# Bissmella/Small-object-detection-transformers

Hardware: AMD Instinct MI355X
Metric: images/sec (1024x1024 RGB+IR) train fwd+bwd (higher is better)
Workload: dtype bf16; 1 GPU; SRyolo_MF.yaml (model.yaml graph), batch 8/GPU @ 1024x1024 RGB+IR, fwd + hand-written bwd + fused SGD-nesterov/weight-decay + EMA step, loss = YOLOv5 ComputeLoss (CIoU + BCE, device kernels), 32 synthetic boxes/image, random-init weights; global_batch=8, parallelism=dp1

## Files before the change

include/sodt_hip.h:

```cpp
#ifndef SODT_HIP_H
#define SODT_HIP_H
#include <stddef.h>
#include <stdint.h>

#ifdef __cplusplus
extern "C" {
#endif

typedef struct ihipStream_t* sodt_stream_t;

#define SODT_OK 0
#define SODT_EINVAL 1
#define SODT_ELAUNCH 2

#define SODT_F32 0
#define SODT_BF16 1
#define SODT_MAX_SEG 9

typedef struct {
  const void* p;
  int ld;
  int klen;
  int dy, dx;
  int mul, shr;
  int Hi, Wi;
} sodt_seg;

typedef struct {
  sodt_seg s[SODT_MAX_SEG];
  int nseg;
  int spatial;
  int Ho, Wo;
} sodt_aspec;

#define SODT_EPI_BIAS 1
#define SODT_EPI_RESID 2
#define SODT_EPI_GELU_DUAL 4
#define SODT_EPI_DGELU 8
#define SODT_EPI_STATS 16
#define SODT_STATS_REPL 16
#define SODT_EPI_AFFINE_SILU 32
#define SODT_EPI_DETECT 64
#define SODT_EPI_OUT_F32 128
#define SODT_EPI_GELU 256
#define SODT_EPI_DGELU_RC 512
#define SODT_EPI_RELU 2048
#define SODT_EPI_DRELU 4096

typedef struct {
  sodt_aspec a;
  const void* W; int ldw;
  void* C; int ldc;
  void* C2; int ldc2;
  const float* bias;
  const void* R; int ldr; int rmod;
  const void* aux; int ldaux;
  double* stats;
  const float* scale; const float* shift;
  int M, N, K, flags;
  int oscatter, omul, ody, odx, OH, OW;
  int det_na, det_no, det_hw;
} sodt_gemm_args;

int sodt_gemm_nt(const sodt_gemm_args* g, int dtype, sodt_stream_t st);
#define SODT_VARIANT_AUTO 0
#define SODT_VARIANT_TILED 1
#define SODT_VARIANT_ASTAT 2
#define SODT_VARIANT_NO_TN3 3
int sodt_gemm_set_variant(int variant);

typedef struct {
  const void* dY; int ldy;
  sodt_aspec x;
  float* dW; int lddw;
  float* dbias;
  int M, N, K;
  int kperm_c, kperm_t;
  int splits;
  float* partial;
  long partial_floats;
} sodt_gemm_tn_args;

int sodt_gemm_tn(const sodt_gemm_tn_args* g, int dtype, sodt_stream_t st);

typedef struct {
  const void* dY; int ldy;
  const void* X; int ldx;
  const void* wT; int ldw;
  const void* aux; int ldaux;
  void* dX; int lddx;
  float* dW; int lddw;
  float* dbias;
  int M, N, K, flags;
  int splits;
  float* partial;
  long partial_floats;
} sodt_linbwd_args;

int sodt_linear_bwd_sq(const sodt_linbwd_args* g, int dtype, sodt_stream_t st);

int sodt_layernorm_fwd(const void* x, const float* gamma, const float* beta, void* y, float* stats,
                       int M, int C, int dtype, sodt_stream_t st);
int sodt_layernorm_bwd(const void* dy, const void* x, const float* stats, const float* gamma,
                       const void* dres, void* dx, float* dgamma, float* dbeta,
                       int M, int C, int dtype, sodt_stream_t st);

int sodt_window_attn_fwd(const void* qkv, const float* bias_t, void* out, float* lse,
                         int B, int H, int W, int C, int heads, int ws, int shift,
                         int dtype, sodt_stream_t st);
int sodt_window_attn_bwd(const void* qkv, const float* bias_t, const void* out, const void* dout,
                         const float* lse, void* dqkv, float* dbias_t, float* dq_acc,
                         int B, int H, int W, int C, int heads, int ws, int shift,
                         int dtype, sodt_stream_t st);

int sodt_window_attn_sp_fwd(const void* qkv, const float* qkv_bias, const float* bias_t, void* out, float* lse,
                            int B, int H, int W, int C, int heads, int ws, int shift, int dtype, sodt_stream_t st);
int sodt_window_attn_sp_bwd(const void* qkv, const float* qkv_bias, const float* bias_t, const void* out, const void* dout,
                            const float* lse, void* dqkv, float* dqkv_bias, float* dbias_t,
                            int B, int H, int W, int C, int heads, int ws, int shift, int dtype, sodt_stream_t st);

int sodt_bilinear_up2_fwd(const void* x, void* y, int ldy, int B, int H, int W, int C, int dtype, sodt_stream_t st);
int sodt_bilinear_up2_bwd(const void* dy, int lddy, void* dx, const void* relu_out, int B, int H, int W, int C, int dtype,
                          sodt_stream_t st);
int sodt_pixel_shuffle2(const void* in, void* out, int B, int H, int W, int C, int inverse, int dtype, sodt_stream_t st);
int sodt_add_rows(void* dst, int ldd, int dcol, const void* src, int lds, int scol, long M, int C, int dtype, sodt_stream_t st);
int sodt_nchw_f32_from_rows(const void* rows, int ld, float* y, int B, int C, int H, int W, int dtype, sodt_stream_t st);
int sodt_rows_from_nchw_f32(const float* y, void* rows, int ld, int B, int C, int H, int W, int dtype, sodt_stream_t st);

int sodt_conv3x3_c64n8_fwd(const void* x, const void* w, const float* bias, void* y, float* y_nchw, int B, int H, int W, int cout, int dtype,
                           sodt_stream_t st);
int sodt_conv3x3_c64n8_dgrad(const void* dy, const float* dy_nchw, const void* wT, void* dx, int B, int H, int W, int cout, int dtype,
                             sodt_stream_t st);
int sodt_conv3x3_c64n8_wgrad(const void* dy, const float* dy_nchw, const void* x, float* dw, float* db, float* scratch, int B, int H, int W,
                             int cout, int dtype, sodt_stream_t st);
long sodt_conv3x3_c64n8_wgrad_scratch_bytes(void);

typedef struct {
  int w_row_stride, w_row_off;
  int in_mul, in_i, in_j;
  int out_mul, out_i, out_j;
} sodt_conv3_geo;
int sodt_conv3x3_c64_fwd(const void* x, const void* w, const float* bias, const void* resid, const void* aux, void* y, int B, int H, int W,
                         int flags, int flip, const sodt_conv3_geo* geo, int dtype, sodt_stream_t st);
int sodt_conv3x3_c64_wgrad(const void* dy, const void* x, float* dw, float* db, float* scratch, int B, int H, int W, const sodt_conv3_geo* geo,
                           int dtype, sodt_stream_t st);
long sodt_conv3x3_c64_wgrad_scratch_bytes(void);

long sodt_wmsa_pack_bytes(int C, int heads, int ws, int dtype);
int sodt_wmsa_pack(const float* qkv_w, const float* qkv_b, const float* proj_w, const float* proj_b,
                   const float* rpb_table, const float* n1_w, const float* n1_b, const float* n2_w,
                   const float* n2_b, void* wpk, int C, int heads, int ws, int dtype, sodt_stream_t st);
// ... 227 lines not shown
```

small-object-detection-transformers_amd/csrc/gemm.hip:

```cpp
#include "gemm_epi.h"
#include "launch.h"
#include "routes.h"

int sodt_nt3_launch(const sodt_gemm_args* g, const NtRoute& r, hipStream_t st);
int sodt_tn3_launch(const sodt_gemm_tn_args* g, const TnRoute& r, hipStream_t st);

namespace {

int g_variant = SODT_VARIANT_AUTO;

constexpr int BM = 128, BN = 128, ROWB = 128;
constexpr int STAGE_BYTES = BM * ROWB;
constexpr int EPI_LD = 132;
constexpr int NT_LDS = BM * EPI_LD * 4;


__device__ __forceinline__ sodt_seg pick_seg(const sodt_aspec& a, int i) {
  sodt_seg s = a.s[0];
#pragma unroll
  for (int j = 1; j < SODT_MAX_SEG; ++j)
    if (i == j) s = a.s[j];
  return s;
}


template <typename T, int CF>
__global__ __launch_bounds__(256, 2) void gemm_nt_kernel(const sodt_gemm_args g) {
  constexpr int KPL = TT<T>::KPL;
  constexpr int BK = 8 * KPL;
  constexpr int SZ = TT<T>::SZ;
  __shared__ __attribute__((aligned(16))) unsigned char smem[NT_LDS];
  unsigned char* sA = smem;
  unsigned char* sB = smem + 2 * STAGE_BYTES;
  __shared__ sodt_seg sSeg[SODT_MAX_SEG];

  const int tid = threadIdx.x, lane = tid & 63, wid = tid >> 6;
  if (tid == 0) {
#pragma unroll
    for (int j = 0; j < SODT_MAX_SEG; ++j) sSeg[j] = g.a.s[j];
  }
  __syncthreads();
  const int wr = wid >> 1, wc = wid & 1;
  const int ntn = (g.N + BN - 1) / BN;
  const int tile = xcd_remap(blockIdx.x, gridDim.x);
  const int tn = tile % ntn, tm = tile / ntn;
  const long m0 = (long)tm * BM;
  const int n0 = tn * BN;

  const int lrow = tid >> 3, lch = tid & 7;
  RowGeo geo[4];
  const int hw = g.a.Ho * g.a.Wo;
#pragma unroll
  for (int i = 0; i < 4; ++i) {
    const long m = m0 + lrow + 32 * i;
    geo[i].ok = m < g.M;
    geo[i].b = 0; geo[i].y = 0; geo[i].x = 0;
    if (g.a.spatial && geo[i].ok) {
      const int b = (int)(m / hw), rem = (int)(m - (long)b * hw);
      geo[i].b = b; geo[i].y = rem / g.a.Wo; geo[i].x = rem - geo[i].y * g.a.Wo;
    }
  }
  int a_seg = 0, a_off = lch * KPL;
  sodt_seg seg = g.a.s[0];
  long srow[4];
#pragma unroll
  for (int i = 0; i < 4; ++i) srow[i] = seg_src_row(seg, geo[i], g.a.spatial, m0 + lrow + 32 * i);

  uint4 ra[4], rb[4];
  const int nk = (g.K + BK - 1) / BK;

  auto load_regs = [&](int kt) {
    while (a_seg < g.a.nseg && a_off >= seg.klen) {
      a_off -= seg.klen;
      ++a_seg;
      if (a_seg < g.a.nseg) {
        seg = sSeg[a_seg];
#pragma unroll
        for (int i = 0; i < 4; ++i) srow[i] = seg_src_row(seg, geo[i], g.a.spatial, m0 + lrow + 32 * i);
      }
    }
    const bool kin = a_seg < g.a.nseg;
    const T* ap = (const T*)seg.p;
#pragma unroll
    for (int i = 0; i < 4; ++i) {
      ra[i] = make_uint4(0, 0, 0, 0);
      if (kin && srow[i] >= 0) ra[i] = *(const uint4*)(ap + srow[i] * seg.ld + a_off);
    }
    a_off += BK;
    const int k = kt * BK + lch * KPL;
    const T* wp = (const T*)g.W;
#pragma unroll
    for (int i = 0; i < 4; ++i) {
      const int n = n0 + lrow + 32 * i;
// ... 800 lines not shown
      }
    }
}

template <typename T>
int launch_tn2(const sodt_gemm_tn_args* g, hipStream_t st) {
  constexpr int lds = 2 * TN2Geo<T>::BMS * (TN2Geo<T>::YROW + TN2Geo<T>::XROW);
  const int tiles = ((g->N + 255) / 256) * ((g->K + 191) / 192);
  return sodt_launch<gemm_tn2_kernel<T>>(dim3(tiles * g->splits), dim3(512), lds, st, *g);
}

bool aspec_ok(const sodt_aspec& a, int K, int kpl) {
  if (a.nseg < 1 || a.nseg > SODT_MAX_SEG) return false;
  long tot = 0;
  for (int i = 0; i < a.nseg; ++i) {
    const sodt_seg& s = a.s[i];
    if (s.klen <= 0 || (s.klen % kpl) || (s.ld % kpl) || (((uintptr_t)s.p) & 15)) return false;
    if (a.spatial && (s.Hi <= 0 || s.Wi <= 0 || s.mul < 1 || s.shr < 0)) return false;
    tot += s.klen;
  }
  if (a.spatial && (a.Ho <= 0 || a.Wo <= 0)) return false;
  return tot == K;
}

#define NT_STATIC_CF(X) \
  X(0) X(SODT_EPI_BIAS) X(SODT_EPI_RESID) X(SODT_EPI_BIAS | SODT_EPI_RESID) X(SODT_EPI_BIAS | SODT_EPI_GELU_DUAL) X(SODT_EPI_DGELU)

template <typename T>
int launch_nt(const sodt_gemm_args* g, const NtRoute& r, hipStream_t st) {
  switch (r.kind) {
    case NT_REFUSED: return SODT_EINVAL;
    case NT_PIPE: return sodt_nt3_launch(g, r, st);
    case NT_BS_STATS: return launch_bs<T, 128, true, -1, false>(g, st);
    case NT_BS_SIMPLE:
      switch (r.cf) {
#define X(F) case F: return launch_bs<T, 128, false, F, true>(g, st);
        NT_STATIC_CF(X)
#undef X
      }
      return SODT_EINVAL;
    case NT_BS_GENERIC: return launch_bs<T, 128, false, -1, false>(g, st);
    case NT_AS128: return launch_as<T, 128>(g, st);
    case NT_AS64: return launch_as<T, 64>(g, st);
    case NT_TILED: {
      const long tiles = ((long)(g->M + BM - 1) / BM) * ((g->N + BN - 1) / BN);
      if (tiles > 0x7fffffffL) return SODT_EINVAL;
      const dim3 grid((unsigned)tiles), block(256);
      switch (r.cf) {
#define X(F) case F: return sodt_launch<gemm_nt_kernel<T, F>>(grid, block, 0, st, *g);
        NT_STATIC_CF(X)
#undef X
      }
      return sodt_launch<gemm_nt_kernel<T, -1>>(grid, block, 0, st, *g);
    }
  }
  return SODT_EINVAL;
}
#undef NT_STATIC_CF

}

extern "C" int sodt_gemm_nt(const sodt_gemm_args* g, int dtype, sodt_stream_t st) {
  if (!g || g->M <= 0 || g->N <= 0 || g->K <= 0 || (dtype != SODT_BF16 && dtype != SODT_F32)) return SODT_EINVAL;
  const int kpl = dtype == SODT_BF16 ? 8 : 4;
  if (!aspec_ok(g->a, g->K, kpl)) return SODT_EINVAL;
  if ((g->ldw % kpl) || (((uintptr_t)g->W) & 15) || !g->C) return SODT_EINVAL;
  if (!(g->flags & SODT_EPI_DETECT)) {
    const int okpl = (g->flags & SODT_EPI_OUT_F32) ? 1 : kpl;
    if ((g->ldc % okpl) || (((uintptr_t)g->C) & 15)) return SODT_EINVAL;
  } else if (g->det_na * g->det_no != g->N || g->det_hw <= 0) return SODT_EINVAL;
  if ((g->flags & SODT_EPI_BIAS) && (!g->bias || (((uintptr_t)g->bias) & 15))) return SODT_EINVAL;
  if ((g->flags & SODT_EPI_RESID) && (!g->R || (g->ldr % kpl))) return SODT_EINVAL;
  if ((g->flags & SODT_EPI_DGELU) && (!g->aux || (g->ldaux % kpl))) return SODT_EINVAL;
  if ((g->flags & SODT_EPI_DRELU) && (!g->aux || (g->ldaux % kpl) || (((uintptr_t)g->aux) & 15) || (g->flags & SODT_EPI_DGELU))) return SODT_EINVAL;
  if ((g->flags & SODT_EPI_GELU_DUAL) && (!g->C2 || (g->ldc2 % kpl))) return SODT_EINVAL;
  if ((g->flags & SODT_EPI_STATS) && !g->stats) return SODT_EINVAL;
  if ((g->flags & SODT_EPI_AFFINE_SILU) && (!g->scale || !g->shift || ((((uintptr_t)g->scale) | ((uintptr_t)g->shift)) & 15))) return SODT_EINVAL;
  if (g->oscatter && !g->a.spatial) return SODT_EINVAL;
  const NtRoute r = nt_route(*g, dtype, g_variant);
  return dtype == SODT_BF16 ? launch_nt<bf16>(g, r, (hipStream_t)st) : launch_nt<float>(g, r, (hipStream_t)st);
}

extern "C" int sodt_gemm_set_variant(int variant) {
  g_variant = variant;
  return SODT_OK;
}

extern "C" int sodt_gemm_tn(const sodt_gemm_tn_args* g, int dtype, sodt_stream_t st) {
  if (!g || g->M <= 0 || g->N <= 0 || g->K <= 0 || g->splits < 1 || !g->dW || !g->dY) return SODT_EINVAL;
  if (dtype != SODT_BF16 && dtype != SODT_F32) return SODT_EINVAL;
  const int kpl = dtype == SODT_BF16 ? 8 : 4;
  if (!aspec_ok(g->x, g->K, kpl)) return SODT_EINVAL;
  if ((g->ldy % kpl) || g->ldy < (g->N + kpl - 1) / kpl * kpl || (((uintptr_t)g->dY) & 15)) return SODT_EINVAL;
  if (g->kperm_t > 1 && (g->kperm_c <= 0 || g->kperm_c * g->kperm_t != g->K)) return SODT_EINVAL;
  const hipStream_t s_ = (hipStream_t)st;
  const TnRoute r = tn_route(*g, dtype, g_variant);
  switch (r.kind) {
    case TN_PIPE: return sodt_tn3_launch(g, r, s_);
    case TN_256x192: return dtype == SODT_BF16 ? launch_tn2<bf16>(g, s_) : launch_tn2<float>(g, s_);
    case TN_TILED: break;
  }
  const int tiles = ((g->N + 127) / 128) * ((g->K + 127) / 128);
  const dim3 grid(tiles * g->splits), block(256);
  return dtype == SODT_BF16 ? sodt_launch<gemm_tn_kernel<bf16>>(grid, block, 0, s_, *g)
                            : sodt_launch<gemm_tn_kernel<float>>(grid, block, 0, s_, *g);
}
```

small-object-detection-transformers_amd/csrc/gemm3.hip:

```cpp
#include "gemm_epi.h"
#include "launch.h"
#include "routes.h"

#ifndef SODT_EXP_PRIO
#define SODT_EXP_PRIO 0
#endif
#if SODT_EXP_PRIO == 1
#define T3_PRIO_HI() __builtin_amdgcn_s_setprio(1)
#define T3_PRIO_LO() __builtin_amdgcn_s_setprio(0)
#else
#define T3_PRIO_HI() do {} while (0)
#define T3_PRIO_LO() do {} while (0)
#endif

namespace {

typedef __attribute__((address_space(3))) void lds_void;
typedef __attribute__((address_space(1))) const void glb_void;
typedef __attribute__((ext_vector_type(4))) unsigned int u32x4;

constexpr int T3_AST = T3_BM * 128;
constexpr int T3_BST = T3_BN * 128;
constexpr int T3_BOFF = 3 * T3_AST;
constexpr int T3_SEGOFF = T3_BOFF + 2 * T3_BST;
// ... 352 lines not shown
          const int n = n0 + wc * 96 + 32 * t + 8 * fg;
          if (PRE || RC) {
            float x[8];
            uint4 pu; pu.x = pre[u][t].x; pu.y = pre[u][t].y; pu.z = pre[u][t].z; pu.w = pre[u][t].w;
            unpack<bf16>(pu, x);
#pragma unroll
            for (int j = 0; j < 8; ++j) {
              if (RC) v[j] *= x[j];
              else if (CF & SODT_EPI_DGELU) v[j] *= dgelu_t<bf16>(x[j]);
              else if (CF & SODT_EPI_DRELU) v[j] = x[j] > 0.f ? v[j] : 0.f;
              else v[j] += x[j];
            }
          }
          if ((CF & SODT_EPI_BIAS) && !RC) {
            const u32x4 b0 = lds_rd128<0>(lbase + T3_BIASOFF + 4 * n), b1 = lds_rd128<16>(lbase + T3_BIASOFF + 4 * n);
            T3_LGKM0();
            v[0] += __uint_as_float(b0.x); v[1] += __uint_as_float(b0.y); v[2] += __uint_as_float(b0.z); v[3] += __uint_as_float(b0.w);
            v[4] += __uint_as_float(b1.x); v[5] += __uint_as_float(b1.y); v[6] += __uint_as_float(b1.z); v[7] += __uint_as_float(b1.w);
          }
          constexpr int CF2 = CF & ~(SODT_EPI_BIAS | SODT_EPI_RESID | SODT_EPI_DGELU | SODT_EPI_DGELU_RC | SODT_EPI_DRELU | SODT_EPI_STATS);
          if constexpr (STATS) {
            if (m < g.M && n < g.N) {
#pragma unroll
              for (int j = 0; j < 8; ++j) { st1[t][j] += v[j]; st2[t][j] = fmaf(v[j], v[j], st2[t][j]); }
            }
          }
          if (m < g.M && n < g.N) {
            if constexpr (OSC) epi_chunk<bf16, -1>(g, CF2, m, n, v, hw);
            else epi_chunk<bf16, CF2>(g, CF2, m, n, v, hw);
          }
          acc[u][t][0] = f32x4{0.f, 0.f, 0.f, 0.f}; acc[u][t][1] = f32x4{0.f, 0.f, 0.f, 0.f};
        }
      }
      c_kt = 0; ++c_ord;
    }
  }
  asm volatile("s_waitcnt vmcnt(0)" ::: "memory");
  if constexpr (STATS) {
    if (wc == 0) {
#pragma unroll
      for (int t = 0; t < NV; ++t)
#pragma unroll
        for (int j = 0; j < 8; ++j) {
          const float a = group16_sum(st1[t][j]), b = group16_sum(st2[t][j]);
          const int n = 32 * t + 8 * fg + j;
          if (fi == 0 && n < g.N) {
            double* st = g.stats + (size_t)((blockIdx.x * 4 + wr) % SODT_STATS_REPL) * 2 * g.N;
            atomicAdd(st + n, (double)a);
            atomicAdd(st + g.N + n, (double)b);
          }
        }
    }
  }
}

template <int CF, bool OSC = false, int NV = 3>
int launch_nt3(const sodt_gemm_args* g, hipStream_t st) {
  const long ntiles = (long)((g->M + T3_BM - 1) / T3_BM) * ((g->N + T3_BN - 1) / T3_BN);
  const int grid = (int)(ntiles < 256 ? ntiles : 256);
  return sodt_launch<gemm_nt3_kernel<CF, OSC, NV>>(dim3(grid), dim3(512), T3_LDS, st, *g);
}


constexpr int N5_ROWS = 32, N5_NST = 5;
constexpr int N5_PST = N5_ROWS * 512;
constexpr int N5_QST = N5_ROWS * 384;
constexpr int N5_STAGE = N5_PST + N5_QST;
constexpr int N5_SEGOFF = N5_NST * N5_STAGE;
constexpr int N5_LDS = N5_SEGOFF + 48 * SODT_MAX_SEG;

template <int OFF> __device__ __forceinline__ uint2 lds_rd_tr(uint32_t addr) {
  typedef __attribute__((ext_vector_type(2))) unsigned int u32x2;
  u32x2 t;
  asm volatile("ds_read_b64_tr_b16 %0, %1 offset:%2" : "=v"(t) : "v"(addr), "n"(OFF));
  uint2 v; v.x = t.x; v.y = t.y;
  return v;
}
template <int HI> __device__ __forceinline__ u32x4 tn3_frag(uint32_t addr) {
  const uint2 lo = lds_rd_tr<0>(addr), hi = lds_rd_tr<HI>(addr);
  u32x4 r; r.x = lo.x; r.y = lo.y; r.z = hi.x; r.w = hi.y;
  return r;
}

struct XDesc { Seg3 sg; int off; int b, y, x; bool colok; const unsigned char* cur; };

template <bool SWAP, bool SPATIAL>
__global__ __launch_bounds__(512) void gemm_tn3_kernel(const sodt_gemm_tn_args g) {
  extern __shared__ __attribute__((aligned(16))) unsigned char dsm[];
  const int tid = threadIdx.x, lane = tid & 63, wid = tid >> 6;
  const int wr = wid >> 1, wc = wid & 1;
  const int fr = lane & 15, fg = lane >> 4;
  const uint32_t lbase = lds_addr(dsm);
#if SODT_EXP_PRIO == 2
  if (__builtin_amdgcn_readfirstlane(threadIdx.x) >= 256) __builtin_amdgcn_s_setprio(1);
#endif
  if (tid == 0) {
#pragma unroll
    for (int j = 0; j < SODT_MAX_SEG; ++j) {
      unsigned char* e = dsm + N5_SEGOFF + 48 * j;
      *(uint64_t*)(e) = (uint64_t)(uintptr_t)g.x.s[j].p;
      *(int4*)(e + 16) = make_int4(g.x.s[j].ld, g.x.s[j].klen, g.x.s[j].dy, g.x.s[j].dx);
      *(int4*)(e + 32) = make_int4(g.x.s[j].mul, g.x.s[j].shr, g.x.s[j].Hi, g.x.s[j].Wi);
    }
  }
  __syncthreads();
  const uint32_t segtab = lbase + N5_SEGOFF;

  const int Pdim = SWAP ? g.K : g.N, Qdim = SWAP ? g.N : g.K;
  const int ntp = (Pdim + 255) / 256, ntq = (Qdim + 191) / 192;
  const int ntiles = ntp * ntq;
  const int lid = xcd_remap(blockIdx.x, gridDim.x);
  const int split = lid / ntiles, tile = lid - split * ntiles;
  const int tq = tile % ntq, tp = tile / ntq;
  const int P0 = tp * 256, Q0 = tq * 192;
  const long rows_per = (((g.M + g.splits - 1) / g.splits) + N5_ROWS - 1) / N5_ROWS * N5_ROWS;
  const long mbeg = (long)split * rows_per;
  const long mend = (mbeg + rows_per < g.M) ? (mbeg + rows_per) : g.M;
  if (mbeg >= mend) return;
  const int nrows = (int)(mend - mbeg);
  const int nsteps = (nrows + N5_ROWS - 1) / N5_ROWS;
  const unsigned char* zero = (const unsigned char*)&g_zero16;
  const int hw = g.x.Ho * g.x.Wo;

  int prow[2], pcol[2], qrow[2], qcol[2];
  const int nq = wid < 4 ? 2 : 1;
#pragma unroll
  for (int e = 0; e < 2; ++e) {
    const int row = 2 * (2 * wid + e) + (lane >> 5), c = lane & 31;
    const int sw = (row & 3) | (((row >> 3) & 1) << 2);
    prow[e] = row; pcol[e] = P0 + (((((c >> 1) ^ sw) << 1) | (c & 1)) << 3);
    const int j = wid < 4 ? 2 * wid + e : 8 + (wid - 4);
    const int id = 64 * j + lane;
    const int r2 = id / 24, c2 = id - r2 * 24;
    const int sw2 = ((r2 >> 1) & 1) | (((r2 >> 3) & 1) << 1);
    qrow[e] = r2; qcol[e] = Q0 + (((((c2 >> 1) ^ sw2) << 1) | (c2 & 1)) << 3);
  }
  const int ycol0 = SWAP ? qcol[0] : pcol[0], ycol1 = SWAP ? qcol[1] : pcol[1];
  const int yrow0 = SWAP ? qrow[0] : prow[0], yrow1 = SWAP ? qrow[1] : prow[1];
  const bool yok0 = ycol0 < g.N, yok1 = ycol1 < g.N;
  const unsigned char* ycur0 = (const unsigned char*)g.dY + (((mbeg + yrow0) * g.ldy + (yok0 ? ycol0 : 0)) << 1);
  const unsigned char* ycur1 = (const unsigned char*)g.dY + (((mbeg + yrow1) * g.ldy + (yok1 ? ycol1 : 0)) << 1);
  const long ystep = (long)N5_ROWS * g.ldy * 2;
  const int xrow0 = SWAP ? prow[0] : qrow[0], xrow1 = SWAP ? prow[1] : qrow[1];
  auto x_setup = [&](XDesc& d, int col, int xrow) {
    d.colok = col < g.K;
    int si = 0;
    if (d.colok) {
      for (int j = 0; j + 1 < g.x.nseg; ++j) {
        const Seg3 t = load_seg3(segtab, si);
        if (col >= t.klen) { col -= t.klen; ++si; }
      }
    }
    d.sg = load_seg3(segtab, d.colok ? si : 0);
    d.off = d.colok ? col : 0;
    const long m = mbeg + xrow;
    d.b = 0; d.y = 0; d.x = 0;
    if (SPATIAL) {
      const int b = (int)(m / hw), rem = (int)(m - (long)b * hw);
      d.b = b; d.y = rem / g.x.Wo; d.x = rem - d.y * g.x.Wo;
    }
    d.cur = d.sg.p + ((m * d.sg.ld + d.off) << 1);
  };
  XDesc xd0, xd1;
  x_setup(xd0, SWAP ? pcol[0] : qcol[0], xrow0);
  x_setup(xd1, SWAP ? pcol[1] : qcol[1], xrow1);
  const long xstep0 = (long)N5_ROWS * xd0.sg.ld * 2, xstep1 = (long)N5_ROWS * xd1.sg.ld * 2;
  int rel = 0;
  auto x_src = [&](const XDesc& d, int xrow) -> const unsigned char* {
    const unsigned char* r = zero;
    if (d.colok && rel + xrow < nrows) {
      if (SPATIAL) {
        const Seg3& sg = d.sg;
        const int yy = d.y * sg.mul + sg.dy, xx = d.x * sg.mul + sg.dx;
        const int yi = yy >> sg.shr, xi = xx >> sg.shr;
        if (yy >= 0 && xx >= 0 && yi < sg.Hi && xi < sg.Wi) {
          const int sr = (d.b * sg.Hi + yi) * sg.Wi + xi;
          r = sg.p + (((long)sr * sg.ld + d.off) << 1);
        }
      } else {
        r = d.cur;
      }
    }
    return r;
  };
  auto x_adv = [&](XDesc& d, long step) {
    if (SPATIAL) {
      d.x += N5_ROWS;
      while (d.x >= g.x.Wo) { d.x -= g.x.Wo; ++d.y; }
      if (d.y >= g.x.Ho) { d.y -= g.x.Ho; ++d.b; }
    } else {
      d.cur += step;
    }
  };
  auto issue = [&](int slot) {
    const uint32_t pdst = slot * N5_STAGE + wid * 2048;
    const uint32_t qdst = slot * N5_STAGE + N5_PST + (wid < 4 ? wid * 2048 : 8192 + (wid - 4) * 1024);
    const unsigned char* sy0 = (yok0 && rel + yrow0 < nrows) ? ycur0 : zero;
    const unsigned char* sy1 = (yok1 && rel + yrow1 < nrows) ? ycur1 : zero;
    const unsigned char* sx0 = x_src(xd0, xrow0);
    const unsigned char* sx1 = x_src(xd1, xrow1);
    __builtin_amdgcn_global_load_lds((glb_void*)(SWAP ? sx0 : sy0), (lds_void*)(dsm + pdst), 16, 0, 0);
    __builtin_amdgcn_global_load_lds((glb_void*)(SWAP ? sx1 : sy1), (lds_void*)(dsm + pdst + 1024), 16, 0, 0);
    __builtin_amdgcn_global_load_lds((glb_void*)(SWAP ? sy0 : sx0), (lds_void*)(dsm + qdst), 16, 0, 0);
    if (nq == 2) __builtin_amdgcn_global_load_lds((glb_void*)(SWAP ? sy1 : sx1), (lds_void*)(dsm + qdst + 1024), 16, 0, 0);
    rel += N5_ROWS;
    ycur0 += ystep; ycur1 += ystep;
    x_adv(xd0, xstep0); x_adv(xd1, xstep1);
  };

  const int q_ = fr >> 2, p_ = fr & 3;
  const int frow = 8 * fg + q_;
  const int swP = q_ | ((fg & 1) << 2);
  const int swQ = (q_ >> 1) | ((fg & 1) << 1);
  uint32_t pa[4], qa[6];
#pragma unroll
  for (int i = 0; i < 4; ++i) pa[i] = lbase + frow * 512 + (((wr * 4 + i) ^ swP) << 5) + 8 * p_;
#pragma unroll
  for (int j = 0; j < 6; ++j) qa[j] = lbase + N5_PST + frow * 384 + (((wc * 6 + j) ^ swQ) << 5) + 8 * p_;

  const bool wave_live = (P0 + wr * 64 < Pdim) && (Q0 + wc * 96 < Qdim);
  const bool do_bias = g.dbias != nullptr && (SWAP ? (tp == 0 && wr == 0) : (tq == 0 && wc == 0)) && wave_live;
  u32x4 ones; ones.x = ones.y = ones.z = ones.w = 0x3F803F80u;

  f32x4 acc[4][6], bacc[6];
#pragma unroll
  for (int i = 0; i < 4; ++i)
#pragma unroll
    for (int j = 0; j < 6; ++j) acc[i][j] = f32x4{0.f, 0.f, 0.f, 0.f};
#pragma unroll
  for (int j = 0; j < 6; ++j) bacc[j] = f32x4{0.f, 0.f, 0.f, 0.f};

  issue(0); issue(1); issue(2); issue(3);
  int slot = 0;
  for (int s = 0; s < nsteps; ++s) {
    if (wid < 4) asm volatile("s_waitcnt vmcnt(12)" ::: "memory");
    else asm volatile("s_waitcnt vmcnt(9)" ::: "memory");
    __builtin_amdgcn_s_barrier();
    asm volatile("" ::: "memory");
    issue(slot == 0 ? N5_NST - 1 : slot - 1);
    if (wave_live) {
      const uint32_t so = slot * N5_STAGE;
      u32x4 fp[4], fq[6];
#pragma unroll
      for (int i = 0; i < 4; ++i) fp[i] = tn3_frag<2048>(pa[i] + so);
#pragma unroll
      for (int j = 0; j < 6; ++j) fq[j] = tn3_frag<1536>(qa[j] + so);
      T3_LGKM0();
      T3_PRIO_HI();
#pragma unroll
      for (int i = 0; i < 4; ++i)
#pragma unroll
        for (int j = 0; j < 6; ++j) mma_sw(acc[i][j], fp[i], fq[j]);
      T3_PRIO_LO();
      if (do_bias) {
        if (SWAP) {
#pragma unroll
          for (int j = 0; j < 6; ++j) mma_sw(bacc[j], ones, fq[j]);
        } else {
#pragma unroll
          for (int i = 0; i < 4; ++i) mma_sw(bacc[i], fp[i], ones);
        }
      }
    }
    slot = slot == N5_NST - 1 ? 0 : slot + 1;
  }
  asm volatile("s_waitcnt vmcnt(0)" ::: "memory");
  __builtin_amdgcn_s_barrier();
  if (!wave_live) return;

  float* part = g.partial ? g.partial + (long)split * g.N * g.K : nullptr;
  if (!SWAP) {
#pragma unroll
    for (int i = 0; i < 4; ++i)
#pragma unroll
      for (int j = 0; j < 6; ++j) {
        const int qc = Q0 + wc * 96 + 16 * j + fr;
        if (qc >= Qdim) continue;
        int k = qc;
        if (g.kperm_t > 1) k = (k % g.kperm_c) * g.kperm_t + k / g.kperm_c;
#pragma unroll
        for (int r = 0; r < 4; ++r) {
          const int n = P0 + wr * 64 + 16 * i + 4 * fg + r;
          if (n < Pdim) {
            if (part) part[(long)n * g.K + qc] = acc[i][j][r];
            else atomicAdd(g.dW + (long)n * g.lddw + k, acc[i][j][r]);
          }
        }
      }
  } else {
    float* patch = (float*)(dsm + wid * (96 * 17 * 4));
#pragma unroll
    for (int i = 0; i < 4; ++i) {
#pragma unroll
      for (int j = 0; j < 6; ++j)
#pragma unroll
        for (int r = 0; r < 4; ++r) patch[(16 * j + fr) * 17 + 4 * fg + r] = acc[i][j][r];
      __builtin_amdgcn_wave_barrier();
      const int pc = P0 + wr * 64 + 16 * i + fr;
      int k = pc;
      if (g.kperm_t > 1) k = (k % g.kperm_c) * g.kperm_t + k / g.kperm_c;
      for (int nn = fg; nn < 96; nn += 4) {
        const int n = Q0 + wc * 96 + nn;
        const float v = patch[nn * 17 + fr];
        if (pc < Pdim && n < Qdim) {
          if (part) part[(long)n * g.K + pc] = v;
          else atomicAdd(g.dW + (long)n * g.lddw + k, v);
        }
      }
      __builtin_amdgcn_wave_barrier();
    }
  }
  if (do_bias) {
    if (SWAP) {
      if (fg == 0) {
#pragma unroll
        for (int j = 0; j < 6; ++j) {
          const int n = Q0 + wc * 96 + 16 * j + fr;
          if (n < g.N) atomicAdd(g.dbias + n, bacc[j][0]);
        }
      }
    } else {
      if (fr == 0) {
#pragma unroll
        for (int i = 0; i < 4; ++i)
#pragma unroll
          for (int r = 0; r < 4; ++r) {
            const int n = P0 + wr * 64 + 16 * i + 4 * fg + r;
            if (n < g.N) atomicAdd(g.dbias + n, bacc[i][r]);
          }
      }
    }
  }
}

__global__ __launch_bounds__(256) void tn3_reduce_kernel(const float* __restrict__ partial, float* __restrict__ dW, int N, int K,
                                                        int lddw, int splits, int kperm_c, int kperm_t) {
  __shared__ float4 red[4][64];
  const long nk4 = (long)N * K / 4;
  const long slice = (long)N * K;
  const int c = threadIdx.x & 63, sg = threadIdx.x >> 6;
  const long i = (long)blockIdx.x * 64 + c;
  float4 a = make_float4(0.f, 0.f, 0.f, 0.f);
  if (i < nk4) {
    const float* p = partial + i * 4;
    int s = sg;
    for (; s + 12 < splits; s += 16) {
      const float4 v0 = *(const float4*)(p + (long)s * slice), v1 = *(const float4*)(p + (long)(s + 4) * slice);
      const float4 v2 = *(const float4*)(p + (long)(s + 8) * slice), v3 = *(const float4*)(p + (long)(s + 12) * slice);
      a.x += (v0.x + v1.x) + (v2.x + v3.x); a.y += (v0.y + v1.y) + (v2.y + v3.y);
      a.z += (v0.z + v1.z) + (v2.z + v3.z); a.w += (v0.w + v1.w) + (v2.w + v3.w);
    }
    for (; s < splits; s += 4) {
      const float4 v = *(const float4*)(p + (long)s * slice);
      a.x += v.x; a.y += v.y; a.z += v.z; a.w += v.w;
    }
  }
  red[sg][c] = a;
  __syncthreads();
  if (sg == 0 && i < nk4) {
    const float4 b1 = red[1][c], b2 = red[2][c], b3 = red[3][c];
    a.x += b1.x + b2.x + b3.x; a.y += b1.y + b2.y + b3.y; a.z += b1.z + b2.z + b3.z; a.w += b1.w + b2.w + b3.w;
    const int n = (int)((i * 4) / K), k0 = (int)((i * 4) - (long)n * K);
    float* d = dW + (long)n * lddw;
    if (kperm_t > 1) {
      const float vv[4] = {a.x, a.y, a.z, a.w};
#pragma unroll
      for (int j = 0; j < 4; ++j) { const int k = k0 + j; d[(k % kperm_c) * kperm_t + k / kperm_c] += vv[j]; }
    } else {
      float4 o = *(float4*)(d + k0);
      o.x += a.x; o.y += a.y; o.z += a.z; o.w += a.w;
      *(float4*)(d + k0) = o;
    }
  }
}

template <bool SWAP, bool SPATIAL>
int launch_tn3(const sodt_gemm_tn_args* g, hipStream_t st) {
  const int Pdim = SWAP ? g->K : g->N, Qdim = SWAP ? g->N : g->K;
  const long tiles = (long)((Pdim + 255) / 256) * ((Qdim + 191) / 192);
  sodt_gemm_tn_args a = *g;
  const bool use_partial = a.partial && a.splits > 1 && (long)a.splits * a.N * a.K <= a.partial_floats &&
                           ((uintptr_t)a.partial & 15) == 0 && (a.lddw % 4) == 0 && ((uintptr_t)a.dW & 15) == 0;
  if (!use_partial) a.partial = nullptr;
  const int rc = sodt_launch<gemm_tn3_kernel<SWAP, SPATIAL>>(dim3((unsigned)(tiles * a.splits)), dim3(512), N5_LDS, st, a);
  if (rc || !use_partial) return rc;
  const long rows_per = ((((long)a.M + a.splits - 1) / a.splits) + N5_ROWS - 1) / N5_ROWS * N5_ROWS;
  const int live = (int)(((long)a.M + rows_per - 1) / rows_per);
  const long nk4 = (long)a.N * a.K / 4;
  const int blocks = (int)((nk4 + 63) / 64);
  return sodt_launch<tn3_reduce_kernel>(dim3(blocks), dim3(256), 0, st, (const float*)a.partial, a.dW, a.N, a.K, a.lddw,
                                        live, a.kperm_c, a.kperm_t);
}

}

int sodt_nt3_launch(const sodt_gemm_args* g, const NtRoute& r, hipStream_t st) {
  if (r.thin) {
    switch (r.cf) {
      case 0: return launch_nt3<0, false, 2>(g, st);
      case SODT_EPI_BIAS: return launch_nt3<SODT_EPI_BIAS, false, 2>(g, st);
      case SODT_EPI_BIAS | SODT_EPI_RESID: return launch_nt3<SODT_EPI_BIAS | SODT_EPI_RESID, false, 2>(g, st);
      case SODT_EPI_RESID: return launch_nt3<SODT_EPI_RESID, false, 2>(g, st);
      case SODT_EPI_BIAS | SODT_EPI_RELU: return launch_nt3<SODT_EPI_BIAS | SODT_EPI_RELU, false, 2>(g, st);
      case SODT_EPI_DRELU: return launch_nt3<SODT_EPI_DRELU, false, 2>(g, st);
      case SODT_EPI_STATS: return launch_nt3<SODT_EPI_STATS, false, 2>(g, st);
      default: return SODT_EINVAL;
    }
  }
  switch (r.cf) {
    case 0: return r.scatter ? launch_nt3<0, true>(g, st) : launch_nt3<0>(g, st);
    case SODT_EPI_BIAS: return launch_nt3<SODT_EPI_BIAS>(g, st);
    case SODT_EPI_RESID: return launch_nt3<SODT_EPI_RESID>(g, st);
    case SODT_EPI_BIAS | SODT_EPI_RESID: return launch_nt3<SODT_EPI_BIAS | SODT_EPI_RESID>(g, st);
    case SODT_EPI_BIAS | SODT_EPI_GELU_DUAL: return launch_nt3<SODT_EPI_BIAS | SODT_EPI_GELU_DUAL>(g, st);
    case SODT_EPI_DGELU: return launch_nt3<SODT_EPI_DGELU>(g, st);
    case SODT_EPI_BIAS | SODT_EPI_GELU: return launch_nt3<SODT_EPI_BIAS | SODT_EPI_GELU>(g, st);
    case SODT_EPI_RELU: return launch_nt3<SODT_EPI_RELU>(g, st);
    case SODT_EPI_BIAS | SODT_EPI_RELU: return launch_nt3<SODT_EPI_BIAS | SODT_EPI_RELU>(g, st);
    case SODT_EPI_DRELU: return launch_nt3<SODT_EPI_DRELU>(g, st);
    case SODT_EPI_BIAS | SODT_EPI_DGELU_RC: return launch_nt3<SODT_EPI_BIAS | SODT_EPI_DGELU_RC>(g, st);
    default: return SODT_EINVAL;
  }
}

int sodt_tn3_launch(const sodt_gemm_tn_args* g, const TnRoute& r, hipStream_t st) {
  if (r.spatial) return r.swap ? launch_tn3<true, true>(g, st) : launch_tn3<false, true>(g, st);
  return r.swap ? launch_tn3<true, false>(g, st) : launch_tn3<false, false>(g, st);
}
```

small-object-detection-transformers_amd/csrc/routes.h:

```cpp
#pragma once
#include "../../include/sodt_hip.h"

constexpr int T3_BM = 256, T3_BN = 192, T3_BK = 64;
constexpr int T3_MAXKLEN = (8192 - 256) / 2;
constexpr int T3_MAXBIAS = 3072;

inline bool nt3_eligible(const sodt_gemm_args& g) {
  switch (g.flags) {
    case 0: case SODT_EPI_BIAS: case SODT_EPI_RESID: case SODT_EPI_BIAS | SODT_EPI_RESID:
    case SODT_EPI_BIAS | SODT_EPI_GELU_DUAL: case SODT_EPI_DGELU: case SODT_EPI_BIAS | SODT_EPI_GELU: break;
    case SODT_EPI_RELU: case SODT_EPI_BIAS | SODT_EPI_RELU: case SODT_EPI_DRELU: break;
    case SODT_EPI_STATS:
      if (g.N > 64 || !g.stats || g.oscatter) return false;
      break;
    case SODT_EPI_BIAS | SODT_EPI_DGELU_RC:
      if (g.K % (2 * T3_BK)) return false;
      break;
    default: return false;
  }
  if (g.rmod > 0 || (g.oscatter && (g.flags != 0 || !g.a.spatial))) return false;
  const int kmin_partial = g.flags == SODT_EPI_STATS ? 192 : 512;
  if (g.N % 8 || (g.N % T3_BN && (g.K < kmin_partial || g.K > T3_MAXKLEN)) || g.K % T3_BK || g.K < 192 || g.M < T3_BM) return false;
  if ((g.flags & SODT_EPI_RESID) && (g.ldr % 8)) return false;
  if ((g.flags & (SODT_EPI_DGELU | SODT_EPI_DRELU)) && (g.ldaux % 8)) return false;
  if ((g.flags & SODT_EPI_BIAS) && g.N > T3_MAXBIAS) return false;
  if ((g.ldw % 8) || (g.ldc % 8)) return false;
  for (int i = 0; i < g.a.nseg; ++i)
    if (g.a.s[i].klen % T3_BK || g.a.s[i].klen > T3_MAXKLEN) return false;
  return true;
}

enum NtKind {
  NT_REFUSED,
  NT_PIPE,
  NT_BS_STATS,
  NT_BS_SIMPLE,
  NT_BS_GENERIC,
  NT_AS128,
  NT_AS64,
  NT_TILED
};
struct NtRoute {
  NtKind kind;
  int cf;
  bool thin;
  bool scatter;
};

inline int nt_static_cf(int flags) {
  switch (flags) {
    case 0: case SODT_EPI_BIAS: case SODT_EPI_RESID: case SODT_EPI_BIAS | SODT_EPI_RESID:
    case SODT_EPI_BIAS | SODT_EPI_GELU_DUAL: case SODT_EPI_DGELU: return flags;
    default: return -1;
  }
}

inline NtRoute nt_route(const sodt_gemm_args& g, int dtype, int variant) {
  const bool bf = dtype == SODT_BF16;
  const bool pipe_ok = bf && nt3_eligible(g);
  if ((g.flags & SODT_EPI_DGELU_RC) && !pipe_ok) return {NT_REFUSED, -1, false, false};
  if (pipe_ok && (variant == SODT_VARIANT_AUTO || variant == SODT_VARIANT_NO_TN3)) {
    bool thin = g.N <= 64 && !g.oscatter;
    switch (g.flags) {
      case 0: case SODT_EPI_BIAS: case SODT_EPI_BIAS | SODT_EPI_RESID: case SODT_EPI_RESID: case SODT_EPI_BIAS | SODT_EPI_RELU:
      case SODT_EPI_DRELU: case SODT_EPI_STATS: break;
      default: thin = false;
    }
    return {NT_PIPE, g.flags, thin, g.oscatter != 0};
  }
  const int kpl = bf ? 8 : 4, KB = g.K * (bf ? 2 : 4);
  if (!(g.flags & SODT_EPI_DETECT) && (KB % 128) == 0 && KB <= 384 && variant != SODT_VARIANT_TILED) {
    const bool relu_resid = (g.flags & (SODT_EPI_RELU | SODT_EPI_DRELU)) && (g.flags & SODT_EPI_RESID);
    if ((g.N % kpl) == 0 && !(g.flags & SODT_EPI_OUT_F32) && variant != SODT_VARIANT_ASTAT && !relu_resid) {
      if (g.flags & SODT_EPI_STATS) return {NT_BS_STATS, -1, false, false};
      const int cf = g.a.nseg == 1 && !g.a.spatial && !g.oscatter ? nt_static_cf(g.flags) : -1;
      return {cf >= 0 ? NT_BS_SIMPLE : NT_BS_GENERIC, cf, false, false};
    }
    return {NT_AS128, -1, false, false};
  }
  return {NT_TILED, g.oscatter ? -1 : nt_static_cf(g.flags), false, false};
}

inline bool tn3_swap(int N, int K) {
  const long a = (long)((N + 255) / 256) * 256 * ((K + 191) / 192) * 192;
  const long b = (long)((K + 255) / 256) * 256 * ((N + 191) / 192) * 192;
  return b < a;
}

enum TnKind {
  TN_PIPE,
  TN_256x192,
  TN_TILED
};
struct TnRoute {
  TnKind kind;
  bool swap, spatial;
};

inline TnRoute tn_route(const sodt_gemm_tn_args& g, int dtype, int variant) {
  if (dtype == SODT_BF16 && variant == SODT_VARIANT_AUTO && (g.N % 8) == 0 && (g.K % 8) == 0 && g.M >= 1024)
    return {TN_PIPE, tn3_swap(g.N, g.K), g.x.spatial != 0};
  if (variant != SODT_VARIANT_TILED && (g.N <= 192 || g.K <= 192))
    return {TN_256x192, false, false};
  return {TN_TILED, false, false};
}

namespace {
struct AttnGeo {
  int B, H, W, C, heads, ws, shift;
  int nwy, nwx, N, nqt;
};
}

inline bool make_geo(AttnGeo& g, int B, int H, int W, int C, int heads, int ws, int shift) {
  if (B <= 0 || H <= 0 || W <= 0 || ws <= 0 || (H % ws) || (W % ws) || heads <= 0 || (C % heads)) return false;
  if ((ws * ws) % 64) return false;
  if (ws < 8 || (64 % ws && ws < 64) ) return false;
  if (ws > 64) return false;
  if (shift < 0 || shift >= ws) return false;
  g.B = B; g.H = H; g.W = W; g.C = C; g.heads = heads; g.ws = ws; g.shift = shift;
  g.nwy = H / ws; g.nwx = W / ws; g.N = ws * ws; g.nqt = g.N / 64;
  return true;
}

constexpr int attn_nw(int dtype, int hd, bool bwd) {
  const int i = hd == 16 ? 0 : hd == 32 ? 1 : hd == 64 ? 2 : -1;
  if (i < 0 || (dtype != SODT_BF16 && dtype != SODT_F32)) return 0;
  constexpr int tab[2][2][3] = {{{4, 2, 2}, {2, 2, 1}},
                                {{4, 4, 2}, {4, 2, 1}}};
  return tab[dtype == SODT_BF16][bwd][i];
}
constexpr int attn_dch(int dtype, int hd) { return hd / (dtype == SODT_BF16 ? 8 : 4); }
constexpr int attn_mma_k(int dtype) { return dtype == SODT_BF16 ? 32 : 16; }
constexpr bool attn_mt1_built(int dtype, int hd) { return attn_dch(dtype, hd) >= 4 && attn_dch(dtype, hd) <= 16; }
constexpr bool attn_mt2_built(int dtype, int hd) { return hd % attn_mma_k(dtype) == 0 && attn_mt1_built(dtype, hd); }

enum AttnFwdKind { AF_FAST, AF_MT2, AF_MT, AF_GENERIC };
enum AttnBwdKind { AB_FAST2, AB_SINGLE, AB_DKV_DQ, AB_MT, AB_GENERIC };
struct AttnRoute {
  int kind;
  int nw;
};

inline AttnRoute attn_fwd_route(int dtype, int hd, const AttnGeo& g) {
  const int nw = attn_nw(dtype, hd, false);
  if (!nw || g.heads % nw) return {AF_GENERIC, 0};
  if (3 * attn_dch(dtype, hd) <= 12 && g.nqt == 1) return {AF_FAST, nw};
  if (g.nqt > 1 && (g.nqt % 4) == 0) {
    if (attn_mt2_built(dtype, hd) && g.shift == 0 && g.ws <= 32) return {AF_MT2, nw};
    if (attn_mt1_built(dtype, hd)) return {AF_MT, nw};
  }
  return {AF_GENERIC, nw};
}

inline AttnRoute attn_bwd_route(int dtype, int hd, const AttnGeo& g) {
  const int nw = attn_nw(dtype, hd, true);
  if (!nw || g.heads % nw) return {AB_GENERIC, 0};
  const bool pfok = 4 * attn_dch(dtype, hd) <= 16;
  if (pfok && g.nqt == 1) return {g.ws == 8 ? AB_FAST2 : AB_SINGLE, nw};
  if (g.nqt == 1) return {AB_GENERIC, nw};
  if (attn_mt2_built(dtype, hd) && g.shift == 0 && g.ws <= 32 && (g.nqt % 4) == 0 && (g.N % 128) == 0)
    return {AB_DKV_DQ, nw};
  return {AB_MT, nw};
}

inline AttnRoute attn_bwd_wm_route(int dtype, int hd, const AttnGeo& g) {
  const int nw = hd == 16 ? attn_nw(dtype, hd, true) : 0;
  if (!nw || g.heads % nw || g.nqt != 1 || g.ws != 8) return {AB_FAST2, 0};
  return {AB_FAST2, nw};
}
inline AttnRoute attn_bwd_rc_route(int dtype, const AttnGeo& g) {
// ... 46 lines not shown
```

small-object-detection-transformers_amd/ops.py:

```python
from __future__ import annotations

import ctypes as C
from typing import List, Optional, Sequence, Tuple

import torch

from . import _lib as L

_lib = L.load()

_active_recorder: Optional[list] = None


class Recorder:

    def __init__(self):
        self.calls: List[Tuple] = []
        self.keep: List = []

    def __enter__(self):
        global _active_recorder
        assert _active_recorder is None, "nested recorders are not supported"
        _active_recorder = self.calls
        return self
# ... 718 lines not shown
def sgd_ema_step_ctl(p, g, mom, ema, p_cast, group_of_chunk, lr, momentum, weight_decay, nesterov, ctl, ema_decay=0.0):
    ng = len(lr)
    arr = lambda v: (C.c_float * ng)(*[float(x) for x in v])
    code = L.F32 if p_cast is None else dt_code(p_cast)
    _launch("sodt_sgd_ema_step_ctl", _p(p), _p(g), _p(mom), _p(ema), _p(p_cast), code, _p(group_of_chunk), p.numel(), ng,
            arr(lr), arr(momentum), arr(weight_decay), int(bool(nesterov)), _p(ctl), C.c_float(ema_decay))


def adam_ema_step_ctl(p, g, exp_avg, exp_avg_sq, ema, p_cast, group_of_chunk, lr, betas, eps, weight_decay, decoupled, ctl,
                      ema_decay=0.0):
    ng = len(lr)
    arr = lambda v: (C.c_double * ng)(*[float(x) for x in v])
    code = L.F32 if p_cast is None else dt_code(p_cast)
    _launch("sodt_adam_ema_step_ctl", _p(p), _p(g), _p(exp_avg), _p(exp_avg_sq), _p(ema), _p(p_cast), code, _p(group_of_chunk),
            p.numel(), ng, arr(lr), arr([b[0] for b in betas]), arr([b[1] for b in betas]), arr(eps), arr(weight_decay),
            int(bool(decoupled)), _p(ctl), C.c_float(ema_decay))


def sr_l1_workspace_bytes(B: int, C_: int, H: int, W: int) -> int:
    return _ws_bytes("sodt_sr_l1_workspace_bytes", int(B), int(C_), int(H), int(W), hint="B * C <= 65535, H * W < 2^31")


def _sr_l1_args(sr, rgb, ir, mode):
    tgt = ir if rgb is None else rgb
    code = L.U8 if tgt.dtype == torch.uint8 else L.F32
    B, Cc, H, W = sr.shape
    return (_p(sr), _p(rgb), _p(ir), code, L.SR_MODES[mode], B, Cc, 0 if rgb is None else rgb.shape[1],
            0 if ir is None else ir.shape[1], H, W)


def sr_l1_fwd(sr, rgb, ir, mode, ws, loss):
    _launch("sodt_sr_l1_fwd", *_sr_l1_args(sr, rgb, ir, mode), _p(ws), ws.numel() * ws.element_size(), _p(loss))


def sr_l1_bwd(sr, rgb, ir, mode, upstream, dsr):
    _launch("sodt_sr_l1_bwd", *_sr_l1_args(sr, rgb, ir, mode), _p(upstream), _p(dsr))


def anchor_stats_workspace_bytes(N: int, S: int) -> int:
    return _ws_bytes("sodt_anchor_stats_workspace_bytes", int(N), int(S))


def anchor_stats(wh, sets, thr_inv, ws, out):
    S, n, _ = sets.shape
    _launch("sodt_anchor_stats", _p(wh), wh.shape[0], _p(sets), S, n, C.c_float(thr_inv), _p(ws),
            ws.numel() * ws.element_size(), _p(out))


def anchor_evolve_workspace_bytes(N: int) -> int:
    return _ws_bytes("sodt_anchor_evolve_workspace_bytes", int(N))


def anchor_evolve(wh, thr_inv, k, f, v, accepted, ws):
    _launch("sodt_anchor_evolve", _p(wh), wh.shape[0], C.c_float(thr_inv), _p(k), k.shape[0], _p(f), _p(v), v.shape[0],
            _p(accepted), _p(ws), ws.numel() * ws.element_size())


def kmeans_lloyd_workspace_bytes(N: int, R: int, n: int) -> int:
    return _ws_bytes("sodt_kmeans_lloyd_workspace_bytes", int(N), int(R), int(n))


def kmeans_lloyd(obs, books, alive, prev, done, thresh, iters, ws):
    R, n, _ = books.shape
    _launch("sodt_kmeans_lloyd", _p(obs), obs.shape[0], _p(books), _p(alive), _p(prev), _p(done), R, n, C.c_double(thresh),
            int(iters), _p(ws), ws.numel() * ws.element_size())


def maxpool5_fwd(x, y, argmax, B, H, W, Cc, ldx=None, ldy=None, x_off=0, y_off=0):
    es = x.element_size()
    _launch("sodt_maxpool5_fwd", x.data_ptr() + x_off * es, x.shape[-1] if ldx is None else ldx, y.data_ptr() + y_off * es,
            y.shape[-1] if ldy is None else ldy, _p(argmax), B, H, W, Cc, dt_code(x))


def maxpool5_bwd(dy, argmax, dx, B, H, W, Cc, lddy=None, lddx=None, dy_off=0, dx_off=0, accumulate=False):
    es = dy.element_size()
    _launch("sodt_maxpool5_bwd", dy.data_ptr() + dy_off * es, dy.shape[-1] if lddy is None else lddy, _p(argmax),
            dx.data_ptr() + dx_off * es, dx.shape[-1] if lddx is None else lddx, int(bool(accumulate)), B, H, W, Cc, dt_code(dy))


def gemm_set_variant(v) -> None:
    _lib.sodt_gemm_set_variant(int(v))


def version() -> str:
    v = _lib.sodt_version().decode()
    ov = L.overrides() if hasattr(L, "overrides") else {}
    return v + (" [" + ", ".join(f"{k}={x}" for k, x in sorted(ov.items())) + "]" if ov else "")
```

Baseline: 216.7 images/sec.

## Double-buffer LDS fragments in TN3 weight-grad GEMM with two-stage issue cadence

Restructures the TN3 weight-gradient GEMM main loop to process two k-steps per iteration. LDS fragment reads for the next stage are double-buffered in registers and overlap with the MFMAs of the current stage. A heuristic-selected 'two-stage' cadence issues global loads two stages ahead with a single barrier per pair, cutting barrier count. It also precomputes row strides with v_xad for spatial address generation and makes the wave id scalar. The cost is higher register pressure from the doubled fragment sets, plus more complex wait-count logic that could mis-synchronise if the counts are wrong.

```diff
diff --git a/include/sodt_hip.h b/include/sodt_hip.h
--- a/include/sodt_hip.h
+++ b/include/sodt_hip.h
@@ -67,6 +67,8 @@
 #define SODT_VARIANT_TILED 1
 #define SODT_VARIANT_ASTAT 2
 #define SODT_VARIANT_NO_TN3 3
+#define SODT_VARIANT_TN3_ONE_STAGE 0x100
+#define SODT_VARIANT_TN3_TWO_STAGE 0x200
 int sodt_gemm_set_variant(int variant);
 
 typedef struct {
diff --git a/small-object-detection-transformers_amd/csrc/gemm.hip b/small-object-detection-transformers_amd/csrc/gemm.hip
--- a/small-object-detection-transformers_amd/csrc/gemm.hip
+++ b/small-object-detection-transformers_amd/csrc/gemm.hip
@@ -8,7 +8,6 @@
 namespace {
 
 int g_variant = SODT_VARIANT_AUTO;
-
 constexpr int BM = 128, BN = 128, ROWB = 128;
 constexpr int STAGE_BYTES = BM * ROWB;
 constexpr int EPI_LD = 132;
@@ -975,7 +974,8 @@
 }
 
 extern "C" int sodt_gemm_set_variant(int variant) {
-  g_variant = variant;
+  g_variant = variant & 0xff;
+  g_tn3_cadence = (variant & SODT_VARIANT_TN3_ONE_STAGE) ? 1 : (variant & SODT_VARIANT_TN3_TWO_STAGE) ? 2 : 0;
   return SODT_OK;
 }
 
diff --git a/small-object-detection-transformers_amd/csrc/gemm3.hip b/small-object-detection-transformers_amd/csrc/gemm3.hip
--- a/small-object-detection-transformers_amd/csrc/gemm3.hip
+++ b/small-object-detection-transformers_amd/csrc/gemm3.hip
@@ -458,12 +458,18 @@
   return r;
 }
 
-struct XDesc { Seg3 sg; int off; int b, y, x; bool colok; const unsigned char* cur; };
+__device__ __forceinline__ uint32_t tn3_xad(uint32_t a, uint32_t b, uint32_t c) {
+  uint32_t r;
+  asm volatile("v_xad_u32 %0, %1, %2, %3" : "=v"(r) : "v"(a), "s"(b), "v"(c));
+  return r;
+}
+
+struct XDesc { Seg3 sg; int off; int b, y, x; bool colok; const unsigned char* cur; unsigned ld2; };
 
 template <bool SWAP, bool SPATIAL>
-__global__ __launch_bounds__(512) void gemm_tn3_kernel(const sodt_gemm_tn_args g) {
+__global__ __launch_bounds__(512) void gemm_tn3_kernel(const sodt_gemm_tn_args g, const int two) {
   extern __shared__ __attribute__((aligned(16))) unsigned char dsm[];
-  const int tid = threadIdx.x, lane = tid & 63, wid = tid >> 6;
+  const int tid = threadIdx.x, lane = tid & 63, wid = __builtin_amdgcn_readfirstlane(tid >> 6);
   const int wr = wid >> 1, wc = wid & 1;
   const int fr = lane & 15, fg = lane >> 4;
   const uint32_t lbase = lds_addr(dsm);
@@ -535,7 +541,8 @@
       const int b = (int)(m / hw), rem = (int)(m - (long)b * hw);
       d.b = b; d.y = rem / g.x.Wo; d.x = rem - d.y * g.x.Wo;
     }
-    d.cur = d.sg.p + ((m * d.sg.ld + d.off) << 1);
+    d.cur = d.sg.p + (((SPATIAL ? 0 : m * d.sg.ld) + d.off) << 1);
+    d.ld2 = (unsigned)d.sg.ld * 2u;
   };
   XDesc xd0, xd1;
   x_setup(xd0, SWAP ? pcol[0] : qcol[0], xrow0);
@@ -551,7 +558,7 @@
         const int yi = yy >> sg.shr, xi = xx >> sg.shr;
         if (yy >= 0 && xx >= 0 && yi < sg.Hi && xi < sg.Wi) {
           const int sr = (d.b * sg.Hi + yi) * sg.Wi + xi;
-          r = sg.p + (((long)sr * sg.ld + d.off) << 1);
+          r = d.cur + (unsigned long)(unsigned)sr * d.ld2;
         }
       } else {
         r = d.cur;
@@ -588,11 +595,8 @@
   const int frow = 8 * fg + q_;
   const int swP = q_ | ((fg & 1) << 2);
   const int swQ = (q_ >> 1) | ((fg & 1) << 1);
-  uint32_t pa[4], qa[6];
-#pragma unroll
-  for (int i = 0; i < 4; ++i) pa[i] = lbase + frow * 512 + (((wr * 4 + i) ^ swP) << 5) + 8 * p_;
-#pragma unroll
-  for (int j = 0; j < 6; ++j) qa[j] = lbase + N5_PST + frow * 384 + (((wc * 6 + j) ^ swQ) << 5) + 8 * p_;
+  const uint32_t pa0 = frow * 512 + (((wr * 4) ^ swP) << 5) + 8 * p_;
+  const uint32_t qa0 = N5_PST + frow * 384 + 8 * p_, qsw = swQ << 5;
 
   const bool wave_live = (P0 + wr * 64 < Pdim) && (Q0 + wc * 96 < Qdim);
   const bool do_bias = g.dbias != nullptr && (SWAP ? (tp == 0 && wr == 0) : (tq == 0 && wc == 0)) && wave_live;
@@ -606,40 +610,70 @@
 #pragma unroll
   for (int j = 0; j < 6; ++j) bacc[j] = f32x4{0.f, 0.f, 0.f, 0.f};
 
+  u32x4 fpA[4], fqA[6], fpB[4], fqB[6];
+#define TN3_VMWAIT(HI, LO)                                                            \
+  do {                                                                                \
+    if (wid < 4) asm volatile("s_waitcnt vmcnt(" #HI ")" ::: "memory");               \
+    else asm volatile("s_waitcnt vmcnt(" #LO ")" ::: "memory");                       \
+    __builtin_amdgcn_s_barrier();                                                     \
+    asm volatile("" ::: "memory");                                                    \
+  } while (0)
+#define TN3_READ(FP, FQ, SLOT)                                                        \
+  do {                                                                                \
+    const uint32_t ps_ = lbase + (SLOT) * N5_STAGE, qs_ = qa0 + ps_;                  \
+    _Pragma("unroll") for (int i = 0; i < 4; ++i) FP[i] = tn3_frag<2048>(tn3_xad(pa0, i << 5, ps_)); \
+    _Pragma("unroll") for (int j = 0; j < 6; ++j) FQ[j] = tn3_frag<1536>(tn3_xad(qsw, (wc * 6 + j) << 5, qs_)); \
+  } while (0)
+#define TN3_MMA(FP, FQ)                                                               \
+  do {                                                                                \
+    T3_PRIO_HI();                                                                     \
+    _Pragma("unroll") for (int i = 0; i < 4; ++i)                                     \
+      _Pragma("unroll") for (int j = 0; j < 6; ++j) mma_sw(acc[i][j], FP[i], FQ[j]);  \
+    T3_PRIO_LO();                                                                     \
+    if (do_bias) {                                                                    \
+      if (SWAP) {                                                                     \
+        _Pragma("unroll") for (int j = 0; j < 6; ++j) mma_sw(bacc[j], ones, FQ[j]);   \
+      } else {                                                                        \
+        _Pragma("unroll") for (int i = 0; i < 4; ++i) mma_sw(bacc[i], FP[i], ones);   \
+      }                                                                               \
+    }                                                                                 \
+  } while (0)
+  auto nx = [](int sl) { return sl == N5_NST - 1 ? 0 : sl + 1; };
   issue(0); issue(1); issue(2); issue(3);
+  if (two) issue(4);
+  TN3_VMWAIT(12, 9);
+  if (!two) issue(4);
+  if (wave_live) TN3_READ(fpA, fqA, 0);
   int slot = 0;
-  for (int s = 0; s < nsteps; ++s) {
-    if (wid < 4) asm volatile("s_waitcnt vmcnt(12)" ::: "memory");
-    else asm volatile("s_waitcnt vmcnt(9)" ::: "memory");
-    __builtin_amdgcn_s_barrier();
-    asm volatile("" ::: "memory");
-    issue(slot == 0 ? N5_NST - 1 : slot - 1);
+  for (int s = 0; s < nsteps; s += 2) {
+    const int s1 = nx(slot), s2 = nx(s1);
+    T3_LGKM0();
+    if (!two) {
+      TN3_VMWAIT(12, 9);
+      issue(slot);
+    }
     if (wave_live) {
-      const uint32_t so = slot * N5_STAGE;
-      u32x4 fp[4], fq[6];
-#pragma unroll
-      for (int i = 0; i < 4; ++i) fp[i] = tn3_frag<2048>(pa[i] + so);
-#pragma unroll
-      for (int j = 0; j < 6; ++j) fq[j] = tn3_frag<1536>(qa[j] + so);
-      T3_LGKM0();
-      T3_PRIO_HI();
-#pragma unroll
-      for (int i = 0; i < 4; ++i)
-#pragma unroll
-        for (int j = 0; j < 6; ++j) mma_sw(acc[i][j], fp[i], fq[j]);
-      T3_PRIO_LO();
-      if (do_bias) {
-        if (SWAP) {
-#pragma unroll
-          for (int j = 0; j < 6; ++j) mma_sw(bacc[j], ones, fq[j]);
-        } else {
-#pragma unroll
-          for (int i = 0; i < 4; ++i) mma_sw(bacc[i], fp[i], ones);
-        }
-      }
-    }
-    slot = slot == N5_NST - 1 ? 0 : slot + 1;
-  }
+      TN3_READ(fpB, fqB, s1);
+      TN3_MMA(fpA, fqA);
+    }
+    T3_LGKM0();
+    if (two) {
+      TN3_VMWAIT(4, 3);
+      issue(slot);
+    } else {
+      TN3_VMWAIT(12, 9);
+    }
+    issue(s1);
+    if (wave_live) {
+      TN3_READ(fpA, fqA, s2);
+      if (s + 1 < nsteps) TN3_MMA(fpB, fqB);
+    }
+    slot = s2;
+  }
+#undef TN3_VMWAIT
+#undef TN3_READ
+#undef TN3_MMA
+  T3_LGKM0();
   asm volatile("s_waitcnt vmcnt(0)" ::: "memory");
   __builtin_amdgcn_s_barrier();
   if (!wave_live) return;
@@ -758,9 +792,10 @@
   const bool use_partial = a.partial && a.splits > 1 && (long)a.splits * a.N * a.K <= a.partial_floats &&
                            ((uintptr_t)a.partial & 15) == 0 && (a.lddw % 4) == 0 && ((uintptr_t)a.dW & 15) == 0;
   if (!use_partial) a.partial = nullptr;
-  const int rc = sodt_launch<gemm_tn3_kernel<SWAP, SPATIAL>>(dim3((unsigned)(tiles * a.splits)), dim3(512), N5_LDS, st, a);
+  const long rows_per = ((((long)a.M + a.splits - 1) / a.splits) + N5_ROWS - 1) / N5_ROWS * N5_ROWS;
+  const int two = g_tn3_cadence ? g_tn3_cadence == 2 : tn3_two_stage(a.N, a.K, SPATIAL, rows_per);
+  const int rc = sodt_launch<gemm_tn3_kernel<SWAP, SPATIAL>>(dim3((unsigned)(tiles * a.splits)), dim3(512), N5_LDS, st, a, two);
   if (rc || !use_partial) return rc;
-  const long rows_per = ((((long)a.M + a.splits - 1) / a.splits) + N5_ROWS - 1) / N5_ROWS * N5_ROWS;
   const int live = (int)(((long)a.M + rows_per - 1) / rows_per);
   const long nk4 = (long)a.N * a.K / 4;
   const int blocks = (int)((nk4 + 63) / 64);
@@ -769,6 +804,8 @@
 }
 
 }
+
+int g_tn3_cadence = 0;
 
 int sodt_nt3_launch(const sodt_gemm_args* g, const NtRoute& r, hipStream_t st) {
   if (r.thin) {
diff --git a/small-object-detection-transformers_amd/csrc/routes.h b/small-object-detection-transformers_amd/csrc/routes.h
--- a/small-object-detection-transformers_amd/csrc/routes.h
+++ b/small-object-detection-transformers_amd/csrc/routes.h
@@ -87,6 +87,11 @@
   return b < a;
 }
 
+inline bool tn3_two_stage(int N, int K, bool spatial, long rows_per) {
+  return rows_per >= 128 && (spatial || (long)N * K >= 500L * (N + K));
+}
+extern int g_tn3_cadence;
+
 enum TnKind {
   TN_PIPE,
   TN_256x192,
diff --git a/small-object-detection-transformers_amd/ops.py b/small-object-detection-transformers_amd/ops.py
--- a/small-object-detection-transformers_amd/ops.py
+++ b/small-object-detection-transformers_amd/ops.py
@@ -824,6 +824,10 @@
     _lib.sodt_gemm_set_variant(int(v))
 
 
+def tn3_set_cadence(c: int) -> None:
+    _lib.sodt_gemm_set_variant({0: 0, 1: 0x100, 2: 0x200}[int(c)])
+
+
 def version() -> str:
     v = _lib.sodt_version().decode()
     ov = L.overrides() if hasattr(L, "overrides") else {}
```

Result: no change. 216.7 images/sec (median of 2 runs) (+0.0%).
